# toverainc/willow-inference-server

Hardware: AMD Instinct MI355X
Metric: realtime_multiple (audio_ms / infer_ms), Whisper large-v2 beam=5, 3.84 s clip (higher is better)
Workload: dtype f16; 1 GPU; whisper-large beam=5 clip=3sec (3840 ms) batch=1/GPU, PCM resident in HBM -> ids on host; parallelism=1 independent replicas (utterance sharding, no data-path collective)

## Files before the change

willow-inference-server_amd/csrc/dec_kernels.hip:

```cpp
#include <string.h>
#include "common.hpp"
#include "kernels.hpp"

namespace wis {

__global__ void pack_gemv_kernel(const f16* __restrict__ W, f16* __restrict__ Wp, int N, int Npad, int K, int n_scale, float scale, int rows) {
  const int ksteps = K / 32;
  const size_t total = (size_t)Npad * ksteps * 4;
  for (size_t idx = (size_t)blockIdx.x * blockDim.x + threadIdx.x; idx < total; idx += (size_t)gridDim.x * blockDim.x) {
    const int row = (int)(idx % rows);
    size_t t = idx / rows;
    const int kq = (int)(t & 3); t >>= 2;
    const int ks = (int)(t % ksteps), nt = (int)(t / ksteps);
    const int n = rows * nt + row, k = 32 * ks + 8 * kq;
    f16x8 v;
    if (n < N) {
      v = *reinterpret_cast<const f16x8*>(W + (size_t)n * K + k);
      if (n < n_scale) {
#pragma unroll
        for (int j = 0; j < 8; ++j) v[j] = (f16)((float)v[j] * scale);
      }
    } else {
#pragma unroll
      for (int j = 0; j < 8; ++j) v[j] = (f16)0.f;
// ... 107 lines not shown
int launch_pack_gemv(hipStream_t st, const f16* W, f16* Wp, int N, int Npad, int K, int n_scale, float scale, int rows) {
  if (K % 32 || Npad % rows || Npad < N || (rows != 16 && rows != 8 && rows != 4)) { set_error("pack_gemv: bad shape N=%d Npad=%d K=%d rows=%d", N, Npad, K, rows); return WIS_E_ARG; }
  const size_t total = (size_t)Npad * (K / 32) * 4;
  int blocks = (int)((total + 255) / 256); if (blocks > 4096) blocks = 4096;
  hipLaunchKernelGGL(pack_gemv_kernel, dim3(blocks), dim3(256), 0, st, W, Wp, N, Npad, K, n_scale, scale, rows);
  return WIS_OK;
}

__global__ void pack_gemv_nc8_kernel(const f16* __restrict__ W, f16* __restrict__ Wp, int N, int Npad, int K) {
  const int kpairs = K / 64;
  const size_t total = (size_t)(Npad / 8) * kpairs * 64;
  for (size_t idx = (size_t)blockIdx.x * blockDim.x + threadIdx.x; idx < total; idx += (size_t)gridDim.x * blockDim.x) {
    const int l = (int)(idx & 63);
    const size_t t = idx >> 6;
    const int kp = (int)(t % kpairs), nt = (int)(t / kpairs);
    const int n = 8 * nt + (l & 7), k = 64 * kp + 32 * ((l >> 3) & 1) + 8 * (l >> 4);
    f16x8 v;
    if (n < N) v = *reinterpret_cast<const f16x8*>(W + (size_t)n * K + k);
    else {
#pragma unroll
      for (int j = 0; j < 8; ++j) v[j] = (f16)0.f;
    }
    *reinterpret_cast<f16x8*>(Wp + idx * 8) = v;
  }
}
int launch_pack_gemv_nc8(hipStream_t st, const f16* W, f16* Wp, int N, int Npad, int K) {
  if (K % 64 || Npad % 8 || Npad < N) { set_error("pack_gemv_nc8: bad shape N=%d Npad=%d K=%d", N, Npad, K); return WIS_E_ARG; }
  const size_t total = (size_t)(Npad / 8) * (K / 64) * 64;
  int blocks = (int)((total + 255) / 256); if (blocks > 4096) blocks = 4096;
  hipLaunchKernelGGL(pack_gemv_nc8_kernel, dim3(blocks), dim3(256), 0, st, W, Wp, N, Npad, K);
  return WIS_OK;
}
bool gemv_nc8_shape(int M, int N, int K) { return (K == 1280 || K == 5120) && N % 8 == 0 && M >= 1 && M <= 16 && M * (K / 8) <= 13 * 256; }

typedef unsigned long long gran_t;
__device__ __forceinline__ void st_gran(gran_t* p, unsigned tag, float v) {
  __hip_atomic_store(p, ((gran_t)tag << 32) | (gran_t)__float_as_uint(v), __ATOMIC_RELAXED, __HIP_MEMORY_SCOPE_AGENT);
}
__device__ __forceinline__ gran_t ld_gran(const gran_t* p) { return __hip_atomic_load(p, __ATOMIC_RELAXED, __HIP_MEMORY_SCOPE_AGENT); }
constexpr unsigned CA_SPIN_LIMIT = 1u << 17;

template <int MB, int MODE, int SC, int RM, bool W8, int NT = 1, int NC = 16>
__device__ __forceinline__ void gemv_body(const GemvP& p, const int KC, const int nt, char* smem) {
  static_assert(NT == 1 || (NT == 2 && MB == 1 && SC > 0), "two-tile workgroups: <= 16 rows, every fragment prefetched");
  static_assert(NC == 16 || (NC == 8 && MB == 1 && NT == 1 && MODE == 2 && SC > 0 && SC % 2 == 0 && !W8), "eight-column tiles: f16 activations and weights, k-steps in pairs, all prefetched");
  typedef typename WFrag<W8>::T WT;
  constexpr int GV_PF = SC > 0 ? (NC == 8 ? SC / 2 : SC) : 16;
  constexpr int rows = NC;
  const int M = p.M, K = p.K;
  const int xstr = KC + 8;
  f16* xs = reinterpret_cast<f16*>(smem);
  float* red = reinterpret_cast<float*>(smem + (((size_t)M * xstr * 2 + 15) & ~(size_t)15));
  float* stats = red + 4 * MB * 64 * 4;
  float* sred = stats + 2 * MAX_ROWS;
  const int tid = threadIdx.x, lane = tid & 63, wave = tid >> 6;
  const int ksteps = K / 32;
  const int S = SC > 0 ? SC : KC / 128;
  const int wt = NT == 2 ? wave >> 1 : 0;
  const int ksl0 = (NT == 2 ? (wave & 1) : wave) * S;
  const bool wact = (lane & 15) < rows;
  const int wstep = 4 * rows;
  const WT* wp4 = NC == 8 ? reinterpret_cast<const WT*>(p.Wp) + ((size_t)nt * (ksteps >> 1) + (ksl0 >> 1)) * 64 + lane
                          : reinterpret_cast<const WT*>(p.Wp) + (size_t)(nt * NT + wt) * ksteps * wstep + (lane >> 4) * rows + (lane & 15);
  const WT wzero = WFrag<W8>::zero();
  const int k4n = K >> 2;
  constexpr bool fast = MODE == 1 || MODE == 3;
// ... 294 lines not shown
template <int MB, int MODE, int SC, int RM, bool W8, int NT = 1, int NC = 16>
__global__ __launch_bounds__(256) void gemv_kernel(WIS_GV_LEAD_DECL(l_), int KC, GemvP p) {
  extern __shared__ __attribute__((aligned(16))) char smem[];
  WIS_GV_LEAD_APPLY(p, l_);
  gemv_body<MB, MODE, SC, RM, W8, NT, NC>(p, KC, blockIdx.x, smem);
}
template <int SCA, int SCB>
__global__ __launch_bounds__(256) void gemv_dual_kernel(int nA, int M, const void* ax, const f16* aWp, const void* bx, const void* bx2, const f16* bWp, int bxsplit,
                                                        GemvP pa, GemvP pb) {
  extern __shared__ __attribute__((aligned(16))) char smem[];
  if ((int)blockIdx.x < nA) { pa.x = ax; pa.x2 = nullptr; pa.Wp = aWp; pa.M = M; pa.K = SCA * 128; gemv_body<1, 2, SCA, 1, false>(pa, SCA * 128, blockIdx.x, smem); }
  else { pb.x = bx; pb.x2 = bx2; pb.Wp = bWp; pb.M = M; pb.K = SCB * 128; pb.xsplit = bxsplit; gemv_body<1, 2, SCB, 1, false>(pb, SCB * 128, (int)blockIdx.x - nA, smem); }
}
int launch_gemv_dual(hipStream_t st, const GemvP& pa, const GemvP& pb) {
  if (pa.M != pb.M || pa.M < 1 || pa.M > 16 || pa.x2 || pa.wscale || pb.wscale || (pa.flags & (GV_LN | GV_QKV)) || (pb.flags & (GV_LN | GV_QKV))) { set_error("gemv_dual: unsupported pair"); return WIS_E_UNSUPPORTED; }
  if (pa.M * (pa.K / 8) > 13 * 256 || pb.M * (pb.K / 8) > 13 * 256 || pa.K % 128 || pb.K % 128) { set_error("gemv_dual: rows do not fit the register staging (M=%d K=%d/%d)", pa.M, pa.K, pb.K); return WIS_E_UNSUPPORTED; }
  const int sa = pa.K / 128, sb = pb.K / 128;
  const size_t aux = (size_t)4 * 64 * 16 + MAX_ROWS * 8 + 4 * 16 * 4 + 16;
  const int Kmax = pa.K > pb.K ? pa.K : pb.K;
  const size_t lds = (((size_t)pa.M * (Kmax + 8) * 2 + 15) & ~(size_t)15) + aux;
  if (lds > 65536) { set_error("gemv_dual: LDS"); return WIS_E_UNSUPPORTED; }
  const int nA = cdiv(pa.N, 16), nB = cdiv(pb.N, 16);
  dim3 grid(nA + nB), block(256);
  GemvP a = pa, b = pb; a.rows = 16; b.rows = 16;
  if (sa == 10 && sb == 20) hipLaunchKernelGGL((gemv_dual_kernel<10, 20>), grid, block, lds, st, nA, a.M, a.x, a.Wp, b.x, b.x2, b.Wp, b.xsplit, a, b);
  else if (sa == 8 && sb == 16) hipLaunchKernelGGL((gemv_dual_kernel<8, 16>), grid, block, lds, st, nA, a.M, a.x, a.Wp, b.x, b.x2, b.Wp, b.xsplit, a, b);
  else if (sa == 6 && sb == 12) hipLaunchKernelGGL((gemv_dual_kernel<6, 12>), grid, block, lds, st, nA, a.M, a.x, a.Wp, b.x, b.x2, b.Wp, b.xsplit, a, b);
  else if (sa == 4 && sb == 8) hipLaunchKernelGGL((gemv_dual_kernel<4, 8>), grid, block, lds, st, nA, a.M, a.x, a.Wp, b.x, b.x2, b.Wp, b.xsplit, a, b);
  else if (sa == 3 && sb == 6) hipLaunchKernelGGL((gemv_dual_kernel<3, 6>), grid, block, lds, st, nA, a.M, a.x, a.Wp, b.x, b.x2, b.Wp, b.xsplit, a, b);
  else { set_error("gemv_dual: K=%d/%d not instantiated", pa.K, pb.K); return WIS_E_UNSUPPORTED; }
  return WIS_OK;
}

int launch_gemv(hipStream_t st, const GemvP& p) {
  if (p.M < 1 || p.M > 16 || p.K % 128 || p.N % 4) { set_error("gemv: M=%d N=%d K=%d unsupported (the LDS-staged form holds one 16-row block; more rows take launch_gemv_frag)", p.M, p.N, p.K); return WIS_E_UNSUPPORTED; }
  int KC = p.K;
  const size_t aux = (size_t)4 * 64 * 16 + MAX_ROWS * 8 + 4 * 16 * 4 + 16;
  while ((size_t)p.M * (KC + 8) * 2 + aux > 65536) {
    int next = 0;
    for (int c = KC - 128; c >= 128; c -= 128) if (p.K % c == 0) { next = c; break; }
    if (!next) { set_error("gemv: cannot chunk K=%d for M=%d", p.K, p.M); return WIS_E_UNSUPPORTED; }
    KC = next;
  }
  const size_t lds = (((size_t)p.M * (KC + 8) * 2 + 15) & ~(size_t)15) + aux;
  const int rows = p.rows ? p.rows : 16;
  GemvP pp = p; pp.rows = rows;
  const int npad = cdiv(p.N, rows) * rows;
  dim3 grid(npad / rows), block(256);
  int mode = 0;
  if (p.flags & GV_LN) {
    if (p.M > 8 || p.K > 2048 || KC != p.K || !p.csum) { set_error("gemv: fused LayerNorm needs M <= 8, K <= 2048 and the folded column sums (M=%d K=%d)", p.M, p.K); return WIS_E_UNSUPPORTED; }
  }
  if (p.flags & GV_LN16) {
    if ((p.flags & GV_LN) || p.M > 8 || p.K > 2048 || p.K % 8 || KC != p.K || !p.csum) {
      set_error("gemv: the LayerNorm fold on f16 rows needs column sums, M <= 8, K <= 2048 (M=%d K=%d)", p.M, p.K); return WIS_E_UNSUPPORTED; }
  }
  if (KC == p.K) {
    if (p.flags & GV_LN) mode = 1;
    else if (p.flags & GV_LN16) mode = 3;
    else if (p.M * (p.K / 8) <= 13 * 256) mode = 2;
  }
  const int sck = KC / 128;
  const int sc = (KC == p.K && (sck == 3 || sck == 4 || sck == 6 || sck == 8 || sck == 10)) ? sck : 0;
#define WIS_GV1(MODEv, SCv, RMv, W8v) hipLaunchKernelGGL((gemv_kernel<1, MODEv, SCv, RMv, W8v>), grid, block, lds, st, WIS_GV_LEAD(pp), KC, pp)
#define WIS_GV(MODEv, SCv, RMv) do { if (p.wscale) WIS_GV1(MODEv, SCv, RMv, true); else WIS_GV1(MODEv, SCv, RMv, false); } while (0)
#define WIS_GV_SC(MODEv, RMv) do { switch (sc) { case 3: WIS_GV(MODEv, 3, RMv); break; case 4: WIS_GV(MODEv, 4, RMv); break; case 6: WIS_GV(MODEv, 6, RMv); break; \
                                                 case 8: WIS_GV(MODEv, 8, RMv); break; case 10: WIS_GV(MODEv, 10, RMv); break; default: WIS_GV(MODEv, 0, RMv); } } while (0)
  if (mode == 1 && sc == 10 && p.M > 3 && p.M <= 5 && !p.wscale && rows == 16 && p.N % 32 == 0 && !(p.flags & (GV_RESID | GV_QKV)) && p.N >= 4096) {
    hipLaunchKernelGGL((gemv_kernel<1, 1, 20, 5, false, 2>), dim3(p.N / 32), block, lds, st, WIS_GV_LEAD(pp), KC, pp);
    return WIS_OK;
  }
  if (rows != 16 && rows != 8) { set_error("gemv: %d-row weight tiles have no kernel", rows); return WIS_E_UNSUPPORTED; }
  if (rows == 8) {
    if (mode != 2 || p.wscale || p.stat_out || (p.flags & GV_QKV) || !gemv_nc8_shape(p.M, p.N, p.K)) {
      set_error("gemv: the eight-column image serves f16 rows and weights at K = 1280 / 5120 without row partials (M=%d N=%d K=%d flags=%d)", p.M, p.N, p.K, p.flags); return WIS_E_UNSUPPORTED; }
    if (sck == 40) hipLaunchKernelGGL((gemv_kernel<1, 2, 40, 1, false, 1, 8>), dim3(p.N / 8), block, lds, st, WIS_GV_LEAD(pp), KC, pp);
    else hipLaunchKernelGGL((gemv_kernel<1, 2, 10, 1, false, 1, 8>), dim3(p.N / 8), block, lds, st, WIS_GV_LEAD(pp), KC, pp);
    return WIS_OK;
  }
  if (mode == 1) { if (p.M <= 3) WIS_GV_SC(1, 3); else if (p.M <= 5) WIS_GV_SC(1, 5); else WIS_GV_SC(1, 8); }
  else if (mode == 3) { if (p.M <= 3) WIS_GV_SC(3, 3); else if (p.M <= 5) WIS_GV_SC(3, 5); else WIS_GV_SC(3, 8); }
  else if (mode == 2) {
    if (sck == 40 && !p.wscale) WIS_GV1(2, 40, 1, false);
    else WIS_GV_SC(2, 1);
  } else WIS_GV_SC(0, 1);
#undef WIS_GV_SC
#undef WIS_GV
#undef WIS_GV1
  return WIS_OK;
}

__device__ __forceinline__ void ln_partials20(const float2* sp, float c, float& s1, float& s2) {
  const float4* sp4 = reinterpret_cast<const float4*>(sp);
  float4 v[10];
#pragma unroll
  for (int i = 0; i < 10; ++i) v[i] = sp4[i];
// ... 2272 lines not shown
```

willow-inference-server_amd/csrc/kernels.hpp:

```cpp
#pragma once
#include "common.hpp"

namespace wis {

struct GemmP {
  const f16* A; int64_t a_bs; int a_rs; int a_rpb;
  const f16* W;
  int M, N, K;
  int klen;
  int n_span = 0, n_period = 0, n_phase = 0;
};
static inline GemmP gemm_plain(const f16* A, int lda, const f16* W, int M, int N, int K) {
  GemmP p; p.A = A; p.a_bs = 0; p.a_rs = lda; p.a_rpb = 0x7fffffff; p.W = W; p.M = M; p.N = N; p.K = K; p.klen = 0; return p;
}
int launch_layernorm(hipStream_t st, const float* x, const float* gamma, const float* beta, f16* y, int M, int d);
int launch_gemm_generic(hipStream_t st, const GemmP& p, const float* bias, const float* resid, void* C, int flags);
int launch_gemm_splitk_resid(hipStream_t st, const GemmP& p, int splits, float* scratch, const float* bias, const float* resid, float* X,
                             const float* ln_gamma = nullptr, const float* ln_beta = nullptr, f16* Y = nullptr);
int launch_gemm_conv1(hipStream_t st, const GemmP& p, const float* bias, f16* C, int T);
int launch_gemm_conv2(hipStream_t st, const GemmP& p, const float* bias, const float* pos, float* X, int T);
int launch_gemm_qkv(hipStream_t st, const GemmP& p, const float* bias, f16* qk, f16* vt, int d, int T, int Tpad, int H);
int launch_gemm_crosskv(hipStream_t st, const GemmP& p, const float* bias, f16* kx, f16* vt, int d, int T, int Tpad, int H, int64_t kx_lstride, int64_t vt_lstride);
int launch_enc_attention(hipStream_t st, const f16* qk, const f16* vt, f16* out, int B, int T, int Tpad, int H, float* part = nullptr, unsigned* counters = nullptr,
                         size_t part_cap = 0);
// ... 25 lines not shown
  const float* wscale;
  void* y;
  int M, N, K, flags;
  float* q; f16* kc; f16* vc; const int* slot; const int* pos; int d; int ctx;
  unsigned long long* prof;
  int rows;
  const void* x2; int xsplit;
  f16* y16;
  int xmb;
  const float* stat_in;
  float* stat_out;
  f16* y_xf;
  int ymb;
  int ksplit; float* kpart; unsigned* kcnt;
  int mb0, mbi;
  int wks, wk0;
};
int launch_gemv(hipStream_t st, const GemvP& p);
int launch_gemv_dual(hipStream_t st, const GemvP& pa, const GemvP& pb);
int launch_gemv_frag(hipStream_t st, const GemvP& p);
int launch_gemv_frag3(hipStream_t st, const GemvP* p, int n);
__host__ __device__ static inline size_t xf_index(int m, int k, int MB) {
  return ((size_t)((k >> 5) * MB + (m >> 4)) * 64 + (m & 15) + 16 * ((k >> 3) & 3)) * 8 + (k & 7);
}
constexpr size_t xf_elems(int K, int MB) { return (size_t)(K / 32) * MB * 64 * 8; }
int launch_xf_pack(hipStream_t st, const void* x, int x_f16, f16* xf, float* stat, int M, int K, int MB);
int launch_dec_embed_xf(hipStream_t st, const f16* emb, const f16* pos_emb, const int* tok, const int* pos, float* x, f16* xf, float* stat, int M, int d, int MB);
int launch_fold_ln(hipStream_t st, f16* W, const float* gamma, const float* beta, float* bias, float* csum, int N, int K, int n_scale, float qscale);
int launch_csum8(hipStream_t st, const f16* W, const float* scale, float* csum, int N, int K, int n_scale, float qscale);
int launch_pack_gemv8(hipStream_t st, const f16* W, unsigned char* Wp, float* scale, int N, int Npad, int K, int n_scale, float qscale);
int launch_pack_gemv(hipStream_t st, const f16* W, f16* Wp, int N, int Npad, int K, int n_scale, float scale, int rows = 16);
int launch_pack_gemv_nc8(hipStream_t st, const f16* W, f16* Wp, int N, int Npad, int K);
bool gemv_nc8_shape(int M, int N, int K);
int gemv_rows_for(int N, int K);

int launch_dec_embed(hipStream_t st, const f16* emb, const f16* pos_emb, const int* tok, const int* pos, float* x, int M, int d, f16* xh = nullptr);
struct SelfAttnP {
  const float* q = nullptr; const f16* kc = nullptr; const f16* vc = nullptr; const int* pos = nullptr; f16* out = nullptr;
  int M = 0, H = 0, d = 0, ctx = 0, rpu = 0, sstride = 0, rmul = 0;
  unsigned long long* prof = nullptr; int out_mb = 0; const int* anc = nullptr; int w0 = 0, aw = 0;
  const int* base = nullptr;
  int nb = 8;
  const int* plen = nullptr;
};
int launch_dec_self_attn(hipStream_t st, const SelfAttnP& p);
constexpr int SA_LONG_MAX_PLEN = 256;
int launch_dec_self_attn_long(hipStream_t st, const float* q, const f16* kc, const f16* vc, const int* pos, const int* plen, int B, int k, int H, int d, int ctx, int sstride,
                              f16* out, int out_mb);
constexpr int CA_SPIN_MAX_BH = 192;
struct CrossAttnP {
  const float* q = nullptr; const f16* kx = nullptr; const f16* vt = nullptr; f16* out = nullptr; float* part = nullptr; unsigned* counters = nullptr;
  int B = 0, R = 0, H = 0, d = 0, T = 0, Tpad = 0, chunks = 0;
  unsigned long long* prof = nullptr; int out_mb = 0;
  const float* xres = nullptr; const float* qcs = nullptr; const float* qb = nullptr;
  unsigned long long* gran = nullptr; unsigned* epoch = nullptr;
  const float* q2 = nullptr; int xres_is_stat = 0;
  int kv_shared = 0;
};
int launch_dec_cross_attn(hipStream_t st, const CrossAttnP& p);

struct SampleCfg {
  int n_vocab, n_vocab_pad, eot, beam, n_cand, max_new, fixed_new, suppress_blank, greedy;
  float length_penalty; int max_hyp; int allow_early_exit; int max_candidates;
  int early_exit_hyps;
};
#ifndef WIS_EARLY_EXIT_NUM_HYPOTHESES
// ... 65 lines not shown
```

willow-inference-server_amd/csrc/model.hip:

```cpp
#include <math.h>
#include <stdlib.h>
#include <string.h>
#include <algorithm>
#include <atomic>
#include <mutex>
#include <memory>
#include <string>
#include <vector>

#include "common.hpp"
#include "kernels.hpp"
#include "model.hpp"

using namespace wis;

namespace wis {

__global__ void convert_kernel(const void* __restrict__ src, int src_f16, void* __restrict__ dst, int dst_f16,
                               int64_t rows, int64_t cols, int64_t dst_ld, int64_t n_scale, float scale) {
  const int64_t total = rows * cols;
  for (int64_t i = (int64_t)blockIdx.x * blockDim.x + threadIdx.x; i < total; i += (int64_t)gridDim.x * blockDim.x) {
    const int64_t r = i / cols, c = i - r * cols;
    float v = src_f16 ? (float)reinterpret_cast<const f16*>(src)[i] : reinterpret_cast<const float*>(src)[i];
    if (r < n_scale) v *= scale;
// ... 160 lines not shown
  WIS_RET(launch_pack_gemv8(st, W, static_cast<unsigned char*>(out), scale_out, N, Npad, K, n_scale, scale));
  if (gamma) WIS_RET(launch_csum8(st, W, scale_out, csum, N, K, n_scale, scale));
  return WIS_OK;
}
static int to_packed(wis_model* m, const Loader& L, const std::string& name, int N, int K, f16* tmp, int n_scale, float scale, const float* ln_gamma, const float* ln_beta,
              float* bias, DecProj* out, int* npad_out = nullptr) {
  TensorSrc s; WIS_RET(L.get(name, N, K, &s));
  const int rows = gemv_rows_for(N, K);
  const int Npad = cdiv(N, rows) * rows;
  hipLaunchKernelGGL(convert_kernel, dim3(blocks_for((int64_t)N * K)), dim3(256), 0, m->st, s.p, s.f16, tmp, 1, (int64_t)N, (int64_t)K, (int64_t)K, (int64_t)0, 1.f);
  float *csum = nullptr, *wscale = nullptr; f16* wp = nullptr;
  if (ln_gamma) { WIS_RET(dalloc(m, &csum, (size_t)Npad)); WIS_HIP_CHECK(hipMemsetAsync(csum, 0, (size_t)Npad * 4, m->st)); }
  if (m->w8) { unsigned char* q8 = nullptr; WIS_RET(dalloc(m, &q8, (size_t)Npad * K)); WIS_RET(dalloc(m, &wscale, (size_t)Npad)); wp = reinterpret_cast<f16*>(q8); }
  else WIS_RET(dalloc(m, &wp, (size_t)Npad * K));
  WIS_RET(prep_projection(m->st, tmp, N, Npad, K, n_scale, scale, ln_gamma, ln_beta, bias, csum, wp, wscale, rows));
  *out = DecProj{wp, wscale, bias, csum, N, K, rows};
  if (npad_out) *npad_out = Npad;
  return WIS_OK;
}
static int load_proj(wis_model* m, const Loader& L, const std::string& name, int N, int K, f16* tmp, int n_scale, float scale, const float* ln_gamma, const float* ln_beta, DecProj* out) {
  float* bias = nullptr;
  if (ln_gamma) WIS_RET(to_f32(m, L, name + "/bias", N, &bias, n_scale, scale));
  WIS_RET(to_packed(m, L, name + "/weight", N, K, tmp, n_scale, scale, ln_gamma, ln_beta, bias, out));
  if (!ln_gamma) { WIS_RET(to_f32(m, L, name + "/bias", N, &bias, n_scale, scale)); out->bias = bias; }
  return WIS_OK;
}

static int add_nc8_image(wis_model* m, const f16* tmp, DecProj* p) {
  if (m->w8 || !gemv_nc8_shape(1, p->N, p->K)) return WIS_OK;
  f16* wp8 = nullptr;
  WIS_RET(dalloc(m, &wp8, (size_t)p->N * p->K));
  WIS_RET(launch_pack_gemv_nc8(m->st, tmp, wp8, p->N, p->N, p->K));
  p->Wp8 = wp8;
  return WIS_OK;
}

int build_cq_fold(hipStream_t st, const f16* wq_gamma, const void* wo, int wo_f16, const float* bo, int d, float qs, f16* fcat, f16* fwot, f16* fwqo, f16* p_cqo, float* b_cqo) {
  hipLaunchKernelGGL(convert_kernel, dim3(blocks_for((int64_t)d * d)), dim3(256), 0, st, wq_gamma, 1, fcat, 1, (int64_t)d, (int64_t)d, (int64_t)2 * d, (int64_t)d, qs);
  hipLaunchKernelGGL(transpose_to_f16_kernel, dim3(cdiv(d, 32), cdiv(d, 32)), dim3(256), 0, st, wo, wo_f16, fwot, d, d);
  GemmP gp = gemm_plain(fcat, 2 * d, fwot, d, d, d);
  WIS_RET(launch_gemm_generic(st, gp, nullptr, nullptr, fwqo, 0));
  hipLaunchKernelGGL(convert_kernel, dim3(blocks_for((int64_t)d * d)), dim3(256), 0, st, fwqo, 1, fcat + d, 1, (int64_t)d, (int64_t)d, (int64_t)2 * d, (int64_t)0, 1.f);
  WIS_RET(launch_pack_gemv(st, fcat, p_cqo, d, d, 2 * d, 0, 1.f, 16));
  hipLaunchKernelGGL(matvec_rows_kernel, dim3(d), dim3(64), 0, st, fcat, 2 * d, bo, b_cqo, d, d);
  return WIS_OK;
}

static int load_weights(wis_model* m, const Loader& L) {
  const wis_config_t& c = m->cfg;
  const int d = c.d_model, V = c.n_vocab;
  const float qs = 0.125f;
  f16* tmp = nullptr;
  f16 *fcat = nullptr, *fwot = nullptr, *fwqo = nullptr;
  {
    size_t big = (size_t)V * d; if ((size_t)4 * d * d > big) big = (size_t)4 * d * d;
    WIS_HIP_CHECK(hipMalloc(reinterpret_cast<void**>(&tmp), big * 2));
    if (m->cq_fold) {
      WIS_HIP_CHECK(hipMalloc(reinterpret_cast<void**>(&fcat), (size_t)2 * d * d * 2));
      WIS_HIP_CHECK(hipMalloc(reinterpret_cast<void**>(&fwot), (size_t)d * d * 2));
      WIS_HIP_CHECK(hipMalloc(reinterpret_cast<void**>(&fwqo), (size_t)d * d * 2));
    }
  }
  int rc = WIS_OK;
  do {
    {
      TensorSrc s;
// ... 49 lines not shown
    float* b_proj = nullptr;
    if ((rc = dalloc(m, &b_proj, (size_t)V + 64))) break;
    if (hipMemsetAsync(b_proj, 0, ((size_t)V + 64) * 4, m->st) != hipSuccess) { set_error("memset failed"); rc = WIS_E_HIP; break; }
    if ((rc = to_packed(m, L, "decoder/embeddings/weight", V, d, tmp, 0, 1.f, m->dec_ln_g, m->dec_ln_b, b_proj, &m->proj, &m->n_vocab_pad))) break;
    m->proj.N = m->n_vocab_pad;
    m->dec.resize(c.n_dec_layers);
    if ((rc = dalloc(m, &m->w_ckv_all, (size_t)c.n_dec_layers * 2 * d * d))) break;
    if ((rc = dalloc(m, &m->b_ckv_all, (size_t)c.n_dec_layers * 2 * d))) break;
    for (int l = 0; l < c.n_dec_layers && !rc; ++l) {
      const std::string p = "decoder/layer_" + std::to_string(l) + "/";
      DecLayerW& w = m->dec[l];
      if ((rc = to_f32(m, L, p + "self_attention/layer_norm/gamma", d, &w.ln1_g))) break;
      if ((rc = to_f32(m, L, p + "self_attention/layer_norm/beta", d, &w.ln1_b))) break;
      if ((rc = load_proj(m, L, p + "self_attention/linear_0", 3 * d, d, tmp, d, qs, w.ln1_g, w.ln1_b, &w.qkv))) break;
      if ((rc = load_proj(m, L, p + "self_attention/linear_1", d, d, tmp, 0, 1.f, nullptr, nullptr, &w.out))) break;
      if ((rc = to_f32(m, L, p + "attention/layer_norm/gamma", d, &w.ln2_g))) break;
      if ((rc = to_f32(m, L, p + "attention/layer_norm/beta", d, &w.ln2_b))) break;
      if ((rc = load_proj(m, L, p + "attention/linear_0", d, d, tmp, d, qs, w.ln2_g, w.ln2_b, &w.cq))) break;
      if (m->cq_fold) {
        TensorSrc so; if ((rc = L.get(p + "self_attention/linear_1/weight", d, d, &so))) break;
        f16* p_cqo = nullptr; float* b_cqo = nullptr;
        if ((rc = dalloc(m, &p_cqo, (size_t)d * 2 * d))) break;
        if ((rc = dalloc(m, &b_cqo, (size_t)d))) break;
        if ((rc = build_cq_fold(m->st, tmp, so.p, so.f16, w.out.bias, d, qs, fcat, fwot, fwqo, p_cqo, b_cqo))) break;
        w.cqo = DecProj{p_cqo, nullptr, b_cqo, nullptr, d, 2 * d, 16};
      }
      w.w_ckv = m->w_ckv_all + (size_t)l * 2 * d * d; w.b_ckv = m->b_ckv_all + (size_t)l * 2 * d;
      if ((rc = to_f16_mat(m, L, p + "attention/linear_1/weight", 2 * d, d, &w.w_ckv))) break;
      if ((rc = to_f32(m, L, p + "attention/linear_1/bias", 2 * d, &w.b_ckv))) break;
      if ((rc = load_proj(m, L, p + "attention/linear_2", d, d, tmp, 0, 1.f, nullptr, nullptr, &w.cout))) break;
      if ((rc = add_nc8_image(m, tmp, &w.cout))) break;
      if ((rc = to_f32(m, L, p + "ffn/layer_norm/gamma", d, &w.ln3_g))) break;
      if ((rc = to_f32(m, L, p + "ffn/layer_norm/beta", d, &w.ln3_b))) break;
      if ((rc = load_proj(m, L, p + "ffn/linear_0", 4 * d, d, tmp, 0, 1.f, w.ln3_g, w.ln3_b, &w.f1))) break;
      if ((rc = load_proj(m, L, p + "ffn/linear_1", d, 4 * d, tmp, 0, 1.f, nullptr, nullptr, &w.f2))) break;
      if ((rc = add_nc8_image(m, tmp, &w.f2))) break;
    }
  } while (0);
  hipError_t e = hipStreamSynchronize(m->st);
  hipFree(tmp); hipFree(fcat); hipFree(fwot); hipFree(fwqo);
  if (rc) return rc;
  if (e != hipSuccess) { set_error("weight conversion failed: %s", hipGetErrorString(e)); return WIS_E_HIP; }
  return WIS_OK;
}

static int frag_ksplit_setting() {
  static const int env_ks = getenv("WIS_FRAG_KSPLIT") ? atoi(getenv("WIS_FRAG_KSPLIT")) : 2;
  return env_ks >= 1 && env_ks <= 8 ? env_ks : 2;
}
int ffn2_ksplit(int K) {
  const int ks = frag_ksplit_setting();
  return ks > 1 && (K / 32) % (4 * ks) == 0 ? ks : 1;
}
void frag_set_ksplit(GemvP& g, int ks, float* part, unsigned* cnt) {
  if (ks > 1) { g.ksplit = ks; g.kpart = part; g.kcnt = cnt; }
}

static int alloc_buffers(wis_model* m) {
  const wis_config_t& c = m->cfg;
  const int d = c.d_model, H = c.n_heads, Bm = c.max_batch, T = c.n_audio_ctx, L = c.n_dec_layers;
  const int slots = Bm * c.max_beam, ctx = c.n_text_ctx;
  m->Tpad = cdiv(T, 64) * 64;
  const size_t img_elems = (size_t)Bm * 3002 * conv1_channels(c.n_mels) + 64;
  WIS_RET(dalloc(m, &m->img, img_elems));
  WIS_RET(dalloc(m, &m->c1, (size_t)Bm * 3002 * d));
  WIS_RET(dalloc(m, &m->x, (size_t)Bm * T * d));
  WIS_RET(dalloc(m, &m->xn, (size_t)Bm * T * d));
  WIS_RET(dalloc(m, &m->qk, (size_t)Bm * T * 2 * d));
  WIS_RET(dalloc(m, &m->vt, (size_t)Bm * H * 64 * m->Tpad));
// ... 210 lines not shown
  const int need = B * m->cfg.n_heads;
  std::atomic<int>& a = g_spin_bh[m->device & 63];
  int cur = a.load(std::memory_order_relaxed);
  while (cur + need <= CA_SPIN_MAX_BH)
    if (a.compare_exchange_weak(cur, cur + need, std::memory_order_relaxed)) { n = need; m->spin_now = true; return; }
}
SpinClaim::~SpinClaim() { if (n) g_spin_bh[m->device & 63].fetch_sub(n, std::memory_order_relaxed); }
void SpinClaim::defer(hipStream_t st) {
  if (!n) return;
  if (hipEventRecord(m->ev[6], st) != hipSuccess) return;
  std::lock_guard<std::mutex> lk(g_spin_mu);
  auto& v = g_spin_deferred[m->device & 63];
  for (auto& d : v) if (d.ev == m->ev[6]) { d.n += n; n = 0; return; }
  v.push_back({m->ev[6], n}); n = 0;
}
int spin_gave_up(wis_model* m, bool* gave_up) {
  int* h = &m->h_pin->giveup;
  WIS_HIP_CHECK(hipMemcpyAsync(h, m->ca_epoch, 4, hipMemcpyDeviceToHost, m->st));
  WIS_HIP_CHECK(hipStreamSynchronize(m->st));
  *gave_up = *h != 0;
  if (*gave_up) {
    WIS_HIP_CHECK(hipMemsetAsync(m->ca_epoch, 0, 4, m->st));
    m->spin_off = true; ++m->handoff_retries;
    fprintf(stderr, "[wis_hip] device %d: decoder cross-attention granule hand-off timed out; this handle uses the ticket hand-off from now on, the call is repeated\n", m->device);
  }
  return WIS_OK;
}


GemvP gemv_small(const DecProj& p, const void* x, void* y, int M, int flags) {
  GemvP g; memset(&g, 0, sizeof(g));
  g.x = x; g.csum = p.csum; g.Wp = p.Wp; g.wscale = p.scale; g.bias = p.bias; g.y = y; g.M = M; g.N = p.N; g.K = p.K; g.flags = flags; g.rows = p.rows;
  if (p.Wp8 && !(flags & ~(GV_RESID | GV_OUT_F32 | GV_GELU)) && gemv_nc8_shape(M, p.N, p.K)) { g.Wp = p.Wp8; g.rows = 8; }
  return g;
}
GemvP gemv_frag(const DecProj& p, const void* xf, int M, int flags) {
  GemvP g; memset(&g, 0, sizeof(g));
  g.x = xf; g.csum = p.csum; g.Wp = p.Wp; g.wscale = p.scale; g.bias = p.bias; g.M = M; g.N = p.N; g.K = p.K; g.flags = flags; g.xmb = cdiv(M, 16); g.rows = 16;
  return g;
}
void out_cq_dual(const DecLayerW& w, const f16* a, const f16* xh, float* x1, float* stat, float* q, int M, GemvP* ga, GemvP* gb) {
  const int d = w.out.K;
  memset(ga, 0, sizeof(*ga));
  ga->x = a; ga->Wp = w.out.Wp; ga->bias = w.out.bias; ga->y = x1; ga->M = M; ga->N = d; ga->K = d; ga->flags = GV_RESID; ga->stat_out = stat;
  memset(gb, 0, sizeof(*gb));
  gb->x = xh; gb->x2 = a; gb->xsplit = d; gb->Wp = w.cqo.Wp; gb->bias = w.cqo.bias; gb->y = q; gb->M = M; gb->N = d; gb->K = w.cqo.K; gb->flags = GV_OUT_F32;
}
void out_cq_frag3(const DecLayerW& w, const f16* af, const f16* xf, float* x1, float* stat, float* q, float* q2, int M, GemvP g3[3]) {
  const int d = w.out.K;
  g3[0] = gemv_frag(w.out, af, M, GV_RESID);
  g3[0].wscale = nullptr; g3[0].y = x1; g3[0].ymb = g3[0].xmb; g3[0].stat_out = stat;
  g3[1] = gemv_frag(w.cqo, xf, M, GV_OUT_F32);
  g3[1].K = d; g3[1].y = q; g3[1].wks = w.cqo.K / 32; g3[1].wk0 = 0;
  g3[2] = gemv_frag(w.cqo, af, M, GV_OUT_F32);
  g3[2].K = d; g3[2].bias = nullptr; g3[2].y = q2; g3[2].wks = w.cqo.K / 32; g3[2].wk0 = d / 32;
}

GemvP frag_resid(const DecProj& p, const f16* xf, float* y, f16* y_xf, float* stat_out, int M) {
  GemvP g = gemv_frag(p, xf, M, GV_RESID);
  g.y = y; g.y_xf = y_xf; g.ymb = g.xmb; g.stat_out = stat_out;
  return g;
}
GemvP frag_ln_f32(const DecProj& p, const f16* xf, const float* stat_in, float* y, int M) {
  GemvP g = gemv_frag(p, xf, M, GV_LN | GV_OUT_F32);
  g.stat_in = stat_in; g.y = y;
  return g;
// ... 435 lines not shown
```

willow-inference-server_amd/csrc/model.hpp:

```cpp
#pragma once
#include <string.h>
#include <array>
#include <atomic>
#include <map>
#include <memory>
#include <vector>

#include "common.hpp"
#include "kernels.hpp"

namespace wis {

struct EncLayerW {
  float *ln1_g, *ln1_b, *ln2_g, *ln2_b;
  f16 *w_qkv, *w_out, *w_f1, *w_f2;
  float *b_qkv, *b_out, *b_f1, *b_f2;
};
struct DecProj {
  const f16* Wp;
  const float* scale;
  const float* bias;
  const float* csum;
  int N, K;
  int rows;
  const f16* Wp8 = nullptr;
};
struct DecLayerW {
  float *ln1_g, *ln1_b, *ln2_g, *ln2_b, *ln3_g, *ln3_b;
  DecProj qkv, out, cq, cout, f1, f2;
  DecProj cqo;
  f16* w_ckv; float* b_ckv;
  std::array<const DecProj*, 6> streamed() const { return {&qkv, &out, &cq, &cout, &f1, &f2}; }
};

struct GraphKey {
  int B, beam, P, max_new, fixed_new, suppress_blank, suppress_default, early_exit, spin, sa_nb; float lp, patience;
  int timestamps, max_init;
  float rep_pen; int rep_ngram;
  int samp_topk; float samp_T; int n_hyp;
  bool operator<(const GraphKey& o) const { return memcmp(this, &o, sizeof(GraphKey)) < 0; }
};

struct WeightSlabs {
  int device; std::vector<void*> slabs; size_t bytes = 0;
  ~WeightSlabs() { hipSetDevice(device); for (void* p : slabs) hipFree(p); }
};

struct AlignState {
  std::vector<int> heads;
  bool ready = false;
  bool capture = false;
  int nsel = 0, sel_cap = 0; size_t sel_bytes = 0;
  std::vector<int> layer_s0;
  int* d_sel_head = nullptr; long long* d_koff = nullptr;
  f16* qsel = nullptr;
  float *W = nullptr, *acc = nullptr;
  unsigned* trace = nullptr; int *rev = nullptr, *path = nullptr, *d_meta = nullptr; float* probs = nullptr;
  int cap_ub0 = 0, cap_t0 = 0, cap_P = 0, last_nmax = 0;
// ... 172 lines not shown
```

willow-inference-server_amd/csrc/taps.hip:

```cpp
#include <string.h>
#include <algorithm>
#include <vector>

#include "common.hpp"
#include "kernels.hpp"
#include "model.hpp"
#include "tap.hpp"

using namespace wis;

extern "C" {

int wis_debug_encode(wis_model_t* m, const float* input, int input_kind, int B, float* enc_out) {
  if (!m || !input || !enc_out) { set_error("wis_debug_encode: bad argument"); return WIS_E_ARG; }
  WIS_ENTER(m, "wis_debug_encode")
  WIS_HIP_CHECK(hipSetDevice(m->device));
  WIS_RET(check_batch(m, B, 1));
  WIS_RET(stage_input(m, input, input_kind, B));
  WIS_RET(run_encoder(m, B));
  const int64_t n = (int64_t)B * m->cfg.n_audio_ctx * m->cfg.d_model;
  launch_f16_to_f32(m->st, m->mem, m->x, n);
  WIS_HIP_CHECK(hipMemcpyAsync(enc_out, m->x, (size_t)n * 4, hipMemcpyDeviceToHost, m->st));
  WIS_HIP_CHECK(hipStreamSynchronize(m->st));
  return WIS_OK;
// ... 289 lines not shown
    xf = xfr; stat_in = stt;
  }
  GemvP g = stage == 0 ? frag_resid(proj, xf, y, reinterpret_cast<f16*>(y_xf), stat_out, M)
          : stage == 1 ? frag_ln_gelu_xf(proj, xf, stat_in, reinterpret_cast<f16*>(y_xf), M) : frag_ln_f32(proj, xf, stat_in, y, M);
  if (xmb) g.xmb = xmb;
  const int ks = ksplit < 0 ? (stage == 0 ? ffn2_ksplit(K) : 1) : ksplit;
  if (ks > 1) {
    const size_t nt = (size_t)cdiv(N, 16);
    float *part = nullptr, *y0 = nullptr; unsigned* cnt = nullptr;
    WIS_RET(t.get(&part, nt * ks * MB * 64 * 4)); WIS_RET(t.get(&cnt, nt, true));
    frag_set_ksplit(g, ks, part, cnt);
    if (stage == 0) { WIS_RET(t.get(&y0, (size_t)M * N)); hipMemcpyAsync(y0, y, (size_t)M * N * 4, hipMemcpyDeviceToDevice, st); }
    WIS_RET(launch_gemv_frag(st, g));
    if (stage == 0) hipMemcpyAsync(y, y0, (size_t)M * N * 4, hipMemcpyDeviceToDevice, st);
  }
  return t.finish(launch_gemv_frag(st, g));
}

int wis_op_dec_embed(int device, const void* emb_f16, const void* pos_f16, const int32_t* tok, const int32_t* pos, float* x, void* xh_f16, void* xf_f16, float* stat,
                     int M, int d, int n_vocab, int n_ctx) {
  Tap t(device, "wis_op_dec_embed"); WIS_RET(t.rc);
  if (!emb_f16 || !pos_f16 || !tok || !pos || !x || M < 1 || M > MAX_ROWS || d < 32 || d % 32 || n_vocab < 1 || n_ctx < 1 || (xf_f16 ? (!stat || xh_f16 != nullptr) : stat != nullptr)) {
    set_error("wis_op_dec_embed: bad argument"); return WIS_E_ARG;
  }
  for (int r = 0; r < M; ++r) if (tok[r] < 0 || tok[r] >= n_vocab || pos[r] < 0 || pos[r] >= n_ctx) { set_error("wis_op_dec_embed: row %d: token %d / position %d out of range", r, tok[r], pos[r]); return WIS_E_ARG; }
  int *d_tok = nullptr, *d_pos = nullptr;
  WIS_RET(t.get(&d_tok, (size_t)M)); WIS_RET(t.get(&d_pos, (size_t)M));
  WIS_HIP_CHECK(hipMemcpy(d_tok, tok, (size_t)M * 4, hipMemcpyHostToDevice)); WIS_HIP_CHECK(hipMemcpy(d_pos, pos, (size_t)M * 4, hipMemcpyHostToDevice));
  const f16 *e = reinterpret_cast<const f16*>(emb_f16), *pe = reinterpret_cast<const f16*>(pos_f16);
  if (xf_f16) return t.finish(launch_dec_embed_xf(t.st, e, pe, d_tok, d_pos, x, reinterpret_cast<f16*>(xf_f16), stat, M, d, cdiv(M, 16)));
  return t.finish(launch_dec_embed(t.st, e, pe, d_tok, d_pos, x, M, d, reinterpret_cast<f16*>(xh_f16)));
}

int wis_op_gemv_cols(int device, const void* x, const void* W, const float* bias, void* y, void* y16, int M, int N, int K, int flags, int cols) {
  Tap t(device, "wis_op_gemv_cols"); WIS_RET(t.rc);
  if (!x || !W || !y || (cols != 8 && cols != 16) || N < 1 || N % cols || (flags & ~(GV_RESID | GV_OUT_F32 | GV_GELU)) || (y16 && !(flags & GV_RESID))) { set_error("wis_op_gemv_cols: bad argument"); return WIS_E_ARG; }
  if (!gemv_nc8_shape(M, N, K)) { set_error("wis_op_gemv_cols: M=%d N=%d K=%d is not a shape of the eight-column form", M, N, K); return WIS_E_UNSUPPORTED; }
  f16* wp = nullptr;
  WIS_RET(t.get(&wp, (size_t)N * K));
  WIS_RET(cols == 8 ? launch_pack_gemv_nc8(t.st, reinterpret_cast<const f16*>(W), wp, N, N, K) : launch_pack_gemv(t.st, reinterpret_cast<const f16*>(W), wp, N, N, K, 0, 1.f, 16));
  GemvP g; memset(&g, 0, sizeof(g));
  g.x = x; g.Wp = wp; g.bias = bias; g.y = y; g.y16 = reinterpret_cast<f16*>(y16); g.M = M; g.N = N; g.K = K; g.flags = flags; g.rows = cols;
  return t.finish(launch_gemv(t.st, g));
}

static int op_dec_self_attn(const char* who, int device, const float* q, const void* kc, const void* vc, const int32_t* pos, void* out,
                            int M, int H, int ctx, int rpu, int sstride, int rmul, int nb, int out_mb, const int32_t* anc, int w0, int aw, const int32_t* base) {
  Tap t(device, who); WIS_RET(t.rc);
  if (!q || !kc || !vc || !pos || !out || M < 1 || H < 1 || rpu < 1 || (nb != 2 && nb != 4 && nb != 8) || (out_mb && out_mb < cdiv(M, 16)) || (base && !anc)) {
    set_error("%s: bad argument", who); return WIS_E_ARG; }
  const int d = 64 * H;
  if (out_mb) WIS_HIP_CHECK(hipMemsetAsync(out, 0, xf_elems(d, out_mb) * 2, t.st));
  SelfAttnP sa;
  sa.q = q; sa.kc = reinterpret_cast<const f16*>(kc); sa.vc = reinterpret_cast<const f16*>(vc); sa.pos = pos; sa.out = reinterpret_cast<f16*>(out);
  sa.M = M; sa.H = H; sa.d = d; sa.ctx = ctx; sa.rpu = rpu; sa.sstride = sstride; sa.rmul = rmul; sa.out_mb = out_mb; sa.anc = anc; sa.w0 = w0; sa.aw = aw; sa.base = base; sa.nb = nb;
  return t.finish(launch_dec_self_attn(t.st, sa));
}
int wis_op_dec_self_attn(int device, const float* q, const void* kc, const void* vc, const int32_t* pos, void* out,
                         int M, int H, int ctx, int rpu, int sstride, int rmul) {
  return op_dec_self_attn("wis_op_dec_self_attn", device, q, kc, vc, pos, out, M, H, ctx, rpu, sstride, rmul, 8, 0, nullptr, 0, 0, nullptr);
}
int wis_op_dec_self_attn_ex(int device, const float* q, const void* kc, const void* vc, const int32_t* pos, void* out,
                            int M, int H, int ctx, int rpu, int sstride, int rmul, int nb, int out_mb,
                            const int32_t* anc, int w0, int aw, const int32_t* base) {
  return op_dec_self_attn("wis_op_dec_self_attn_ex", device, q, kc, vc, pos, out, M, H, ctx, rpu, sstride, rmul, nb, out_mb, anc, w0, aw, base);
}
int wis_op_dec_self_attn_long(int device, const float* q, const void* kc, const void* vc, const int32_t* pos, const int32_t* plen, void* out,
                              int B, int k, int H, int ctx, int out_mb) {
  Tap t(device, "wis_op_dec_self_attn_long"); WIS_RET(t.rc);
// ... 232 lines not shown
```

Before: 151.3 x realtime.

## Add five-column GEMV image for decoder FFN down-projection at K=5120

```diff
diff --git a/willow-inference-server_amd/csrc/dec_kernels.hip b/willow-inference-server_amd/csrc/dec_kernels.hip
--- a/willow-inference-server_amd/csrc/dec_kernels.hip
+++ b/willow-inference-server_amd/csrc/dec_kernels.hip
@@ -163,6 +163,44 @@
   return WIS_OK;
 }
 bool gemv_nc8_shape(int M, int N, int K) { return (K == 1280 || K == 5120) && N % 8 == 0 && M >= 1 && M <= 16 && M * (K / 8) <= 13 * 256; }
+
+__global__ void pack_gemv_nc5_kernel(const f16* __restrict__ W, f16* __restrict__ Wp, int N, int K, int kw) {
+  const int rq = (kw + 2) / 3, nr = K / 32 / kw;
+  const size_t total = (size_t)(N / 5) * nr * rq * 64;
+  for (size_t idx = (size_t)blockIdx.x * blockDim.x + threadIdx.x; idx < total; idx += (size_t)gridDim.x * blockDim.x) {
+    const int l = (int)(idx & 63);
+    size_t t = idx >> 6;
+    const int u = (int)(t % rq); t /= rq;
+    const int rg = (int)(t % nr), slab = (int)(t / nr);
+    const int row = l & 15, j = row / 5, ksl = 3 * u + j;
+    const int n = 5 * slab + (row - 5 * j), k = 32 * (rg * kw + ksl) + 8 * (l >> 4);
+    f16x8 v;
+    if (row < 15 && ksl < kw) v = *reinterpret_cast<const f16x8*>(W + (size_t)n * K + k);
+    else {
+#pragma unroll
+      for (int e = 0; e < 8; ++e) v[e] = (f16)0.f;
+    }
+    *reinterpret_cast<f16x8*>(Wp + idx * 8) = v;
+  }
+}
+size_t gemv_nc5_elems(int N, int K, int kw) { return (size_t)(N / 5) * (K / 32 / kw) * ((kw + 2) / 3) * 512; }
+int launch_pack_gemv_nc5(hipStream_t st, const f16* W, f16* Wp, int N, int K, int kw) {
+  if (N < 5 || N % 5 || K % 32 || kw < 1 || (K / 32) % kw) { set_error("pack_gemv_nc5: bad shape N=%d K=%d kw=%d", N, K, kw); return WIS_E_ARG; }
+  const size_t total = gemv_nc5_elems(N, K, kw) / 8;
+  int blocks = (int)((total + 255) / 256); if (blocks > 4096) blocks = 4096;
+  hipLaunchKernelGGL(pack_gemv_nc5_kernel, dim3(blocks), dim3(256), 0, st, W, Wp, N, K, kw);
+  return WIS_OK;
+}
+static int device_cu_count() {
+  static int cus[64];
+  int dev = 0;
+  if (hipGetDevice(&dev) != hipSuccess || dev < 0 || dev >= 64) return 0;
+  if (!cus[dev]) { int v = 0; if (hipDeviceGetAttribute(&v, hipDeviceAttributeMultiprocessorCount, dev) != hipSuccess) v = 0; cus[dev] = v > 0 ? v : -1; }
+  return cus[dev] > 0 ? cus[dev] : 0;
+}
+bool gemv_nc5_shape(int M, int N, int K, int flags) {
+  return K == 5120 && M >= 1 && M * (K / 8) <= 13 * 256 && N >= 5 && N % 5 == 0 && !(flags & ~(GV_RESID | GV_OUT_F32 | GV_GELU)) && N / 5 <= device_cu_count();
+}
 
 typedef unsigned long long gran_t;
 __device__ __forceinline__ void st_gran(gran_t* p, unsigned tag, float v) {
@@ -523,8 +561,97 @@
   return WIS_OK;
 }
 
+#define GV_IN_ORDER() __builtin_amdgcn_sched_barrier(0x104)
+template <int CTRL>
+__device__ __forceinline__ f16x8 nc5_rot(const u32x4& w) {
+  u32x4 r;
+#pragma unroll
+  for (int e = 0; e < 4; ++e) r[e] = (unsigned)__builtin_amdgcn_update_dpp(0, (int)w[e], CTRL, 0xf, 0xf, false);
+  return *reinterpret_cast<const f16x8*>(&r);
+}
+__device__ __forceinline__ f32x4 ld4_f32(const float* p) { f32x4 v; __builtin_memcpy(&v, p, 16); return v; }
+__device__ __forceinline__ f32x4 add4_f32(const f32x4& a, const f32x4& b) { return f32x4{a[0] + b[0], a[1] + b[1], a[2] + b[2], a[3] + b[3]}; }
+__device__ __forceinline__ void st_nc5_f32(float* p, const f32x4& v, int kq) { if (kq) p[3] = v[3]; else __builtin_memcpy(p, &v, 16); }
+__device__ __forceinline__ void st_nc5_f16(f16* p, const f32x4& v, int kq) {
+  const f16x4 h = {(f16)v[0], (f16)v[1], (f16)v[2], (f16)v[3]};
+  if (kq) p[3] = h[3]; else __builtin_memcpy(p, &h, 8);
+}
+template <int SC>
+__global__ __launch_bounds__(256) void gemv_nc5_kernel(WIS_GV_LEAD_DECL(l_), int KC, GemvP p) {
+  extern __shared__ __attribute__((aligned(16))) char smem[];
+  WIS_GV_LEAD_APPLY(p, l_);
+  (void)KC;
+  constexpr int K = SC * 128, RQ = (SC + 2) / 3, xstr = K + 8, c8 = K / 8, NXH = 13;
+  const int M = p.M;
+  f16* xs = reinterpret_cast<f16*>(smem);
+  float* red = reinterpret_cast<float*>(smem + (((size_t)M * xstr * 2 + 15) & ~(size_t)15));
+  const int tid = threadIdx.x, lane = tid & 63, wave = tid >> 6, slab = blockIdx.x;
+  unsigned long long* pf = (slab == 0 && tid == 0) ? p.prof : nullptr;
+  if (tid == 0) tl_begin(p.prof);
+  stamp(pf, 0);
+  u32x4 xh[NXH];
+  const int nx = M * c8;
+  const u32x4* x8 = reinterpret_cast<const u32x4*>(p.x);
+#pragma unroll
+  for (int i = 0; i < NXH; ++i) { const int idx = tid + 256 * i; if (idx < nx) xh[i] = x8[idx]; }
+  const u32x4* wp4 = reinterpret_cast<const u32x4*>(p.Wp) + ((size_t)slab * 4 + wave) * RQ * 64 + lane;
+  u32x4 wf[RQ];
+#pragma unroll
+  for (int u = 0; u < RQ; ++u) { wf[u] = __builtin_nontemporal_load(wp4 + (size_t)u * 64); GV_IN_ORDER(); }
+  stamp(pf, 1);
+#pragma unroll
+  for (int i = 0; i < NXH; ++i) {
+    const int idx = tid + 256 * i;
+    if (idx < nx) { const int row = idx / c8, k8 = idx - row * c8; *reinterpret_cast<u32x4*>(xs + (size_t)row * xstr + k8 * 8) = xh[i]; }
+  }
+  __syncthreads();
+  stamp(pf, 3);
+  f32x4 acc = f32x4{0.f, 0.f, 0.f, 0.f};
+  const int m = lane & 15, kq = lane >> 4;
+  const f16* xw = xs + (m < M ? m : M - 1) * xstr + 8 * kq + wave * SC * 32;
+  f16x8 xb[SC];
+#pragma unroll
+  for (int k = 0; k < SC; ++k) xb[k] = *reinterpret_cast<const f16x8*>(xw + k * 32);
+  __builtin_amdgcn_sched_barrier(0);
+#pragma unroll
+  for (int u = 0; u < RQ; ++u) {
+    acc = __builtin_amdgcn_mfma_f32_16x16x32_f16(*reinterpret_cast<const f16x8*>(&wf[u]), xb[3 * u], acc, 0, 0, 0);
+    if (3 * u + 1 < SC) acc = __builtin_amdgcn_mfma_f32_16x16x32_f16(nc5_rot<0x12B>(wf[u]), xb[3 * u + 1 < SC ? 3 * u + 1 : 0], acc, 0, 0, 0);
+    if (3 * u + 2 < SC) acc = __builtin_amdgcn_mfma_f32_16x16x32_f16(nc5_rot<0x126>(wf[u]), xb[3 * u + 2 < SC ? 3 * u + 2 : 0], acc, 0, 0, 0);
+    GV_IN_ORDER();
+  }
+  stamp(pf, 4);
+  const bool ep_ok = wave == 0 && m < M && kq < 2;
+  const size_t o = (size_t)m * p.N + 5 * slab + kq;
+  f32x4 ep_bias = f32x4{0.f, 0.f, 0.f, 0.f}, ep_res = ep_bias;
+  if (ep_ok) {
+    if (p.bias) ep_bias = ld4_f32(p.bias + 5 * slab + kq);
+    if (p.flags & GV_RESID) ep_res = ld4_f32(reinterpret_cast<const float*>(p.y) + o);
+  }
+  *reinterpret_cast<f32x4*>(red + ((size_t)wave * 64 + lane) * 4) = acc;
+  __syncthreads();
+  stamp(pf, 5);
+  if (wave == 0) {
+    f32x4 s = f32x4{0.f, 0.f, 0.f, 0.f};
+#pragma unroll
+    for (int w = 0; w < 4; ++w) s = add4_f32(s, *reinterpret_cast<const f32x4*>(red + ((size_t)w * 64 + lane) * 4));
+    if (ep_ok) {
+      if (kq) s[3] = s[0];
+      s = add4_f32(s, ep_bias);
+      if (p.flags & GV_GELU) { s[0] = gelu_erf(s[0]); s[1] = gelu_erf(s[1]); s[2] = gelu_erf(s[2]); s[3] = gelu_erf(s[3]); }
+      if (p.flags & GV_RESID) {
+        const f32x4 r = add4_f32(ep_res, s);
+        st_nc5_f32(reinterpret_cast<float*>(p.y) + o, r, kq);
+        if (p.y16) st_nc5_f16(p.y16 + o, r, kq);
+      } else if (p.flags & GV_OUT_F32) st_nc5_f32(reinterpret_cast<float*>(p.y) + o, s, kq);
+      else st_nc5_f16(reinterpret_cast<f16*>(p.y) + o, s, kq);
+    }
+  }
+  stamp(pf, 6);
+  if (tid == 0) tl_end(p.prof);
+}
 int launch_gemv(hipStream_t st, const GemvP& p) {
-  if (p.M < 1 || p.M > 16 || p.K % 128 || p.N % 4) { set_error("gemv: M=%d N=%d K=%d unsupported (the LDS-staged form holds one 16-row block; more rows take launch_gemv_frag)", p.M, p.N, p.K); return WIS_E_UNSUPPORTED; }
+  if (p.M < 1 || p.M > 16 || p.K % 128 || (p.N % 4 && p.rows != 5)) { set_error("gemv: M=%d N=%d K=%d unsupported (the LDS-staged form holds one 16-row block; more rows take launch_gemv_frag)", p.M, p.N, p.K); return WIS_E_UNSUPPORTED; }
   int KC = p.K;
   const size_t aux = (size_t)4 * 64 * 16 + MAX_ROWS * 8 + 4 * 16 * 4 + 16;
   while ((size_t)p.M * (KC + 8) * 2 + aux > 65536) {
@@ -553,6 +680,12 @@
   }
   const int sck = KC / 128;
   const int sc = (KC == p.K && (sck == 3 || sck == 4 || sck == 6 || sck == 8 || sck == 10)) ? sck : 0;
+  if (rows == 5) {
+    if (mode != 2 || p.wscale || p.stat_out || p.x2 || !gemv_nc5_shape(p.M, p.N, p.K, p.flags)) {
+      set_error("gemv: the five-column image serves f16 rows and weights at K = 5120 without row partials, one dispatch round (M=%d N=%d K=%d flags=%d)", p.M, p.N, p.K, p.flags); return WIS_E_UNSUPPORTED; }
+    hipLaunchKernelGGL((gemv_nc5_kernel<40>), dim3(p.N / 5), block, lds, st, WIS_GV_LEAD(pp), KC, pp);
+    return WIS_OK;
+  }
 #define WIS_GV1(MODEv, SCv, RMv, W8v) hipLaunchKernelGGL((gemv_kernel<1, MODEv, SCv, RMv, W8v>), grid, block, lds, st, WIS_GV_LEAD(pp), KC, pp)
 #define WIS_GV(MODEv, SCv, RMv) do { if (p.wscale) WIS_GV1(MODEv, SCv, RMv, true); else WIS_GV1(MODEv, SCv, RMv, false); } while (0)
 #define WIS_GV_SC(MODEv, RMv) do { switch (sc) { case 3: WIS_GV(MODEv, 3, RMv); break; case 4: WIS_GV(MODEv, 4, RMv); break; case 6: WIS_GV(MODEv, 6, RMv); break; \
diff --git a/willow-inference-server_amd/csrc/kernels.hpp b/willow-inference-server_amd/csrc/kernels.hpp
--- a/willow-inference-server_amd/csrc/kernels.hpp
+++ b/willow-inference-server_amd/csrc/kernels.hpp
@@ -81,6 +81,9 @@
 int launch_pack_gemv(hipStream_t st, const f16* W, f16* Wp, int N, int Npad, int K, int n_scale, float scale, int rows = 16);
 int launch_pack_gemv_nc8(hipStream_t st, const f16* W, f16* Wp, int N, int Npad, int K);
 bool gemv_nc8_shape(int M, int N, int K);
+size_t gemv_nc5_elems(int N, int K, int kw);
+int launch_pack_gemv_nc5(hipStream_t st, const f16* W, f16* Wp, int N, int K, int kw);
+bool gemv_nc5_shape(int M, int N, int K, int flags);
 int gemv_rows_for(int N, int K);
 
 int launch_dec_embed(hipStream_t st, const f16* emb, const f16* pos_emb, const int* tok, const int* pos, float* x, int M, int d, f16* xh = nullptr);
diff --git a/willow-inference-server_amd/csrc/model.hip b/willow-inference-server_amd/csrc/model.hip
--- a/willow-inference-server_amd/csrc/model.hip
+++ b/willow-inference-server_amd/csrc/model.hip
@@ -216,6 +216,15 @@
   WIS_RET(dalloc(m, &wp8, (size_t)p->N * p->K));
   WIS_RET(launch_pack_gemv_nc8(m->st, tmp, wp8, p->N, p->N, p->K));
   p->Wp8 = wp8;
+  return WIS_OK;
+}
+static int add_nc5_image(wis_model* m, const f16* tmp, DecProj* p, bool* added) {
+  *added = false;
+  if (m->w8 || !gemv_nc5_shape(1, p->N, p->K, GV_RESID)) return WIS_OK;
+  f16* wp5 = nullptr;
+  WIS_RET(dalloc(m, &wp5, gemv_nc5_elems(p->N, p->K, 40)));
+  WIS_RET(launch_pack_gemv_nc5(m->st, tmp, wp5, p->N, p->K, 40));
+  p->Wp5 = wp5; *added = true;
   return WIS_OK;
 }
 
@@ -331,9 +340,11 @@
       if ((rc = add_nc8_image(m, tmp, &w.cout))) break;
       if ((rc = to_f32(m, L, p + "ffn/layer_norm/gamma", d, &w.ln3_g))) break;
       if ((rc = to_f32(m, L, p + "ffn/layer_norm/beta", d, &w.ln3_b))) break;
+      bool nc5 = false;
       if ((rc = load_proj(m, L, p + "ffn/linear_0", 4 * d, d, tmp, 0, 1.f, w.ln3_g, w.ln3_b, &w.f1))) break;
       if ((rc = load_proj(m, L, p + "ffn/linear_1", d, 4 * d, tmp, 0, 1.f, nullptr, nullptr, &w.f2))) break;
-      if ((rc = add_nc8_image(m, tmp, &w.f2))) break;
+      if ((rc = add_nc5_image(m, tmp, &w.f2, &nc5))) break;
+      if (!nc5 && (rc = add_nc8_image(m, tmp, &w.f2))) break;
     }
   } while (0);
   hipError_t e = hipStreamSynchronize(m->st);
@@ -610,6 +621,7 @@
   GemvP g; memset(&g, 0, sizeof(g));
   g.x = x; g.csum = p.csum; g.Wp = p.Wp; g.wscale = p.scale; g.bias = p.bias; g.y = y; g.M = M; g.N = p.N; g.K = p.K; g.flags = flags; g.rows = p.rows;
   if (p.Wp8 && !(flags & ~(GV_RESID | GV_OUT_F32 | GV_GELU)) && gemv_nc8_shape(M, p.N, p.K)) { g.Wp = p.Wp8; g.rows = 8; }
+  if (p.Wp5 && !p.scale && !p.csum && gemv_nc5_shape(M, p.N, p.K, flags)) { g.Wp = p.Wp5; g.rows = 5; }
   return g;
 }
 GemvP gemv_frag(const DecProj& p, const void* xf, int M, int flags) {
diff --git a/willow-inference-server_amd/csrc/model.hpp b/willow-inference-server_amd/csrc/model.hpp
--- a/willow-inference-server_amd/csrc/model.hpp
+++ b/willow-inference-server_amd/csrc/model.hpp
@@ -24,6 +24,7 @@
   int N, K;
   int rows;
   const f16* Wp8 = nullptr;
+  const f16* Wp5 = nullptr;
 };
 struct DecLayerW {
   float *ln1_g, *ln1_b, *ln2_g, *ln2_b, *ln3_g, *ln3_b;
diff --git a/willow-inference-server_amd/csrc/taps.hip b/willow-inference-server_amd/csrc/taps.hip
--- a/willow-inference-server_amd/csrc/taps.hip
+++ b/willow-inference-server_amd/csrc/taps.hip
@@ -345,9 +345,33 @@
   return t.finish(launch_dec_embed(t.st, e, pe, d_tok, d_pos, x, M, d, reinterpret_cast<f16*>(xh_f16)));
 }
 
+static int op_gemv_cols5(Tap& t, const void* x, const void* W, const float* bias, void* y, void* y16, int M, int N, int K, int flags, bool w8) {
+  const int Npad = cdiv(N, 16) * 16;
+  f16 *wp = nullptr, *wrow = nullptr, *wp5 = nullptr; float *wsc = nullptr, *b2 = nullptr;
+  WIS_RET(t.get(&wp, (size_t)Npad * K)); WIS_RET(t.get(&wrow, (size_t)N * K)); WIS_RET(t.get(&b2, (size_t)Npad, true));
+  if (w8) WIS_RET(t.get(&wsc, (size_t)Npad));
+  hipMemcpyAsync(wrow, W, (size_t)N * K * 2, hipMemcpyDeviceToDevice, t.st);
+  if (bias) hipMemcpyAsync(b2, bias, (size_t)N * 4, hipMemcpyDeviceToDevice, t.st);
+  WIS_RET(prep_projection(t.st, wrow, N, Npad, K, 0, 1.f, nullptr, nullptr, b2, nullptr, wp, wsc, 16));
+  DecProj proj{wp, wsc, bias ? b2 : nullptr, nullptr, N, K, 16};
+  if (!w8 && gemv_nc5_shape(1, N, K, flags)) {
+    WIS_RET(t.get(&wp5, gemv_nc5_elems(N, K, 40)));
+    WIS_RET(launch_pack_gemv_nc5(t.st, wrow, wp5, N, K, 40));
+    proj.Wp5 = wp5;
+  }
+  GemvP g = gemv_small(proj, x, y, M, flags);
+  g.y16 = reinterpret_cast<f16*>(y16);
+  return t.finish(launch_gemv(t.st, g));
+}
 int wis_op_gemv_cols(int device, const void* x, const void* W, const float* bias, void* y, void* y16, int M, int N, int K, int flags, int cols) {
   Tap t(device, "wis_op_gemv_cols"); WIS_RET(t.rc);
-  if (!x || !W || !y || (cols != 8 && cols != 16) || N < 1 || N % cols || (flags & ~(GV_RESID | GV_OUT_F32 | GV_GELU)) || (y16 && !(flags & GV_RESID))) { set_error("wis_op_gemv_cols: bad argument"); return WIS_E_ARG; }
+  const bool w8 = cols == 5 && (flags & 32);
+  if (w8) flags &= ~32;
+  if (!x || !W || !y || (cols != 5 && cols != 8 && cols != 16) || N < 1 || (cols != 5 && N % cols) || (flags & ~(GV_RESID | GV_OUT_F32 | GV_GELU)) || (y16 && !(flags & GV_RESID))) { set_error("wis_op_gemv_cols: bad argument"); return WIS_E_ARG; }
+  if (cols == 5) {
+    if (M < 1 || M > 16 || K < 128 || K % 128) { set_error("wis_op_gemv_cols: M=%d K=%d", M, K); return WIS_E_ARG; }
+    return op_gemv_cols5(t, x, W, bias, y, y16, M, N, K, flags, w8);
+  }
   if (!gemv_nc8_shape(M, N, K)) { set_error("wis_op_gemv_cols: M=%d N=%d K=%d is not a shape of the eight-column form", M, N, K); return WIS_E_UNSUPPORTED; }
   f16* wp = nullptr;
   WIS_RET(t.get(&wp, (size_t)N * K));
```

Measured after the change: 153.1 x realtime (median of 6 runs). 1.01x the previous value.
